# google-deepmind/mujoco_mpc

Measured on NVIDIA H100. Metric: env-steps/sec, higher is better.
Workload: dtype f32

## Files before the change

### mujoco_mpc_b200/csrc/dev_data.cuh

```cuda
#pragma once
#include <cuda_runtime.h>

#include "dev_model.h"

#ifndef MJPC_NO_COMPACT
#define MJPC_COMPACT 1
#endif
#ifdef MJPC_COMPACT
#define MJPC_ROLL _Pragma("unroll 1")
#define MJPC_HESS_ROLLED 1
#else
#define MJPC_ROLL
#endif

namespace mjpc_dev {

constexpr int kMaxSplinePoints = 64;
#define MJPC_D_ARRAYS(X)                                                                                          \
  X(qpos, M.nq) X(qvel, M.nv) X(ctrl, M.nu) X(qacc, M.nv) X(qacc_warmstart, M.nv) X(mocap_pos, 3 * M.nmocap)      \
  X(mocap_quat, 4 * M.nmocap) X(xpos, 3 * M.nbody) X(xquat, 4 * M.nbody) X(xmat, 9 * M.nbody)                     \
  X(xipos, 3 * M.nbody) X(ximat, 9 * M.nbody) X(xanchor, 3 * M.njnt) X(xaxis, 3 * M.njnt)                         \
  X(geom_xpos, 3 * M.ngeom) X(geom_xmat, 9 * M.ngeom) X(site_xpos, 3 * M.nsite) X(subtree_com, 3 * M.nbody)       \
  X(cinert, 10 * M.nbody) X(crb, 10 * M.nbody) X(cdof, 6 * M.nv) X(cdof_dot, 6 * M.nv) X(cvel, 6 * M.nbody)       \
  X(cacc, 6 * M.nbody) X(cfrc, 6 * M.nbody) X(cfrc_sub, 6 * M.nbody) X(subtree_linvel, 3 * M.nbody)               \
// ... 54 lines not shown
  int hdr;
  int lay;
  int ibase;
  int dbase;
  int lane;
  int ncon, nefc, nitem, niter, nlim;
  int ndrow;
  const float* gkey;
  int xfrc_on;
  int npseudo;
  int warn;
  float time;
  unsigned* sync;
  int sync_slot;
  int sync_mode;
#ifdef MJPC_PHASE_TIMING
  long long tph[8], tlast;
#endif
};
#ifdef MJPC_PHASE_TIMING
#define PHASE(c, i) do { const long long t_ = clock64(); (c).tph[i] += t_ - (c).tlast; (c).tlast = t_; } while (0)
#else
#define PHASE(c, i) do { } while (0)
#endif
template <int V> struct IntC { static constexpr int v = V; };
constexpr int kHdrWords = (int)((sizeof(DevModel) + 15) / 16) * 4;
constexpr int kLayWords = (int)((sizeof(DevLayout) + 15) / 16) * 4;

struct DynSpec {
  static constexpr bool kStatic = false;
  static constexpr int kNV = 0, kNHPair = 0;
  static constexpr int kWide = 1, kTask = 0;
  static __device__ __forceinline__ const DevModel& hdr(const Ctx& c) { return *reinterpret_cast<const DevModel*>(g_smem + c.hdr); }
  static __device__ __forceinline__ const DevModel& model(const Ctx& c) { return hdr(c); }
  template <int ID> static __device__ __forceinline__ float* mf(const Ctx& c) { return g_smem + hdr(c).fo[ID]; }
  template <int ID> static __device__ __forceinline__ int* mi(const Ctx& c) {
    return reinterpret_cast<int*>(g_smem + c.ibase) + hdr(c).io[ID];
  }
  template <int ID> static __device__ __forceinline__ float* df(const Ctx& c) {
// ... 22 lines not shown
  template <int ID> static __device__ __forceinline__ int* mi(const Ctx&) {
    return reinterpret_cast<int*>(g_smem) + IntC<View::nf + w(offsetof(DevModel, io), ID)>::v;
  }
  template <int ID> static __device__ __forceinline__ float* df(const Ctx&) {
    return g_smem + IntC<kData0 + K::kLayoutOff[ID]>::v;
  }
};

#define CM(c) (SP::hdr(c))
#define MF(n) (SP::template mf<F_##n>(c))
#define MI(n) (SP::template mi<I_##n>(c))
#define DF(n) (SP::template df<D_##n>(c))
#define DI(n) (reinterpret_cast<int*>(SP::template df<D_##n>(c)))

enum { WIDE_EXIT = 0, WIDE_HESSIAN = 1 };
struct WideBox { int cmd, ncon, nlim, ndrow, nefc; int task_exit, task_warn; float task_cost; };
__device__ __forceinline__ WideBox& wide_box() { __shared__ WideBox box; return box; }
template <class SP>
__device__ __forceinline__ void wide_bar() {
  if constexpr (SP::kWide > 1) asm volatile("bar.sync 1, %0;" ::"n"(32 * SP::kWide) : "memory");
  else __syncwarp();
}
__device__ __forceinline__ void task_bar() { asm volatile("bar.sync 2, 64;" ::: "memory"); }
template <class SP> __device__ __forceinline__ int wide_lane(const Ctx& c) { return SP::kWide > 1 ? (int)threadIdx.x : c.lane; }
template <class SP>
__device__ __forceinline__ void wide_post(const Ctx& c, int cmd) {
  if constexpr (SP::kWide > 1) {
    WideBox& b = wide_box();
    if (c.lane == 0) { b.cmd = cmd; b.ncon = c.ncon; b.nlim = c.nlim; b.ndrow = c.ndrow; b.nefc = c.nefc; }
    wide_bar<SP>();
  }
}

#ifndef MJPC_PAIR_TIMEOUT
#define MJPC_PAIR_TIMEOUT 400000
#endif
constexpr long long kPairTimeout = MJPC_PAIR_TIMEOUT;
__device__ __forceinline__ unsigned ld_vol(const unsigned* p) {
  unsigned v;
  asm volatile("ld.volatile.global.u32 %0, [%1];" : "=r"(v) : "l"(p) : "memory");
  return v;
}
__device__ __forceinline__ void st_vol(unsigned* p, unsigned v) { asm volatile("st.volatile.global.u32 [%0], %1;" ::"l"(p), "r"(v) : "memory"); }
__device__ __forceinline__ void pair_sync_init(Ctx& c, unsigned* table, int mode) {
  c.sync = nullptr; c.sync_slot = -1; c.sync_mode = mode;
// ... 272 lines not shown
```

### mujoco_mpc_b200/csrc/dev_physics.cuh

```cuda
#pragma once
#include "dev_data.cuh"

namespace mjpc_dev {



template <class SP>
__device__ __noinline__ void k_kinematics(Ctx& c) {
  auto&& M = SP::model(c);
  const int lane = c.lane;
  float *xpos = DF(xpos), *xquat = DF(xquat), *xmat = DF(xmat), *xipos = DF(xipos), *ximat = DF(ximat);
  float *xanchor = DF(xanchor), *xaxis = DF(xaxis);
  const float* qpos = DF(qpos);
  if (lane < 3) { xpos[lane] = 0; xipos[lane] = 0; }
  if (lane < 4) xquat[lane] = lane == 0 ? 1.f : 0.f;
  if (lane < 9) { float v = (lane % 4 == 0) ? 1.f : 0.f; xmat[lane] = v; ximat[lane] = v; }
  __syncwarp();
  const int *level_adr = MI(level_adr), *level_body = MI(level_body), *parentid = MI(body_parentid),
            *mocapid = MI(body_mocapid), *jntadr = MI(body_jntadr), *jntnum = MI(body_jntnum),
            *jtype = MI(jnt_type), *jqadr = MI(jnt_qposadr);
  const float *bpos = MF(body_pos), *bquat = MF(body_quat), *bipos = MF(body_ipos), *biquat = MF(body_iquat),
              *jpos = MF(jnt_pos), *jaxis = MF(jnt_axis), *qpos0 = MF(qpos0);
  for (int l = 0; l < M.nlevel; l++) {
    const int a = level_adr[l], e = level_adr[l + 1];
// ... 1108 lines not shown
          FOR_DIM(j, 1, dim) hw[i + j] = Dm * c1 * fr[j - 1] * fr[j - 1];
          float* q = xw + 36 * ci;
          q[0] = mu; q[6] = 0.f;
          FOR_DIM(j, 1, dim) { q[j] = -fr[j - 1] * mu * u[j] * iT; q[6 + j] = fr[j - 1] * u[j]; }
          q[12] = Dm;
          q[13] = Dm * (mu * N * iT * iT * iT - mu * mu * iT * iT);
        }
      }
    }
  }
  cost = warp_sum(cost);
  __syncwarp();
  return cost;
}

template <class SP, int NV, int NQ>
__device__ __forceinline__ void hessian_dense_reg(Ctx& c) {
  auto&& M = SP::model(c);
  const int lane = wide_lane<SP>(c);
  constexpr int WN = 32 * SP::kWide;
  constexpr int NVP = (NV + 3) / 4 * 4;
  const float *qM = DF(qM), *hw = DF(efc_hw), *Jd = DF(efc_Jd), *Xd = DF(efc_Xd), *xw = DF(efc_hc);
  float* H = DF(qH);
  const int *frow = MI(floss_row), *edof = DI(efc_dof), *state = DI(efc_state), *cadr = DI(con_adr),
            *hi = MI(hpair_i), *hj = MI(hpair_j), *cside = DI(con_side), *cdim = DI(con_dim);
  const int NE = M.nhpair, ncon = c.ncon;
  float* Wc = DF(efc_blk);
  float* g = DF(dofbuf);
  const float* W6 = DF(efc_w);
  {
    float* xwm = DF(efc_hc);
    MJPC_ROLL
    for (int w = lane; w < ncon * 6; w += WN) {
      const int ci = w / 6, p = w - 6 * ci;
      const int a0 = cadr[ci];
      float v = 0.f, u = 0.f;
      if (a0 >= 0 && cside[ci] != 0 && state[a0] == STATE_CONE) {
        const int dim = cdim[ci];
        const float* q = xw + 36 * ci;
        FOR_DIM(a, 0, dim) { const float wa = W6[6 * (a0 + a) + p]; v += q[a] * wa; u += q[6 + a] * wa; }
      }
      xwm[36 * ci + 14 + p] = v; xwm[36 * ci + 20 + p] = u;
    }
    wide_bar<SP>();
    constexpr int kMaxRows = 10;
    const bool pyr = M.cone == CONE_PYRAMIDAL;
    const int nwork = ncon * 21;
    MJPC_ROLL
    for (int base = 0; base < nwork; base += WN) {
      const int w = min(base + lane, nwork - 1);
      const int ci = w / 21, e = w - 21 * ci;
      const int p = (e >= 1) + (e >= 3) + (e >= 6) + (e >= 10) + (e >= 15);
      const int q2 = e - p * (p + 1) / 2;
      const int a0r = cadr[ci];
      const bool on = a0r >= 0 && cside[ci] != 0;
      const int a0 = max(a0r, 0);
      const int nrows = on ? cdim[ci] : 0;
      float acc = 0.f;
#ifdef MJPC_HESS_ROLLED
#pragma unroll 1
#else
#pragma unroll
#endif
      for (int a = 0; a < kMaxRows; a++) {
        if (a >= 6 && !pyr) break;
        const int r = min(a0 + a, M.maxefc - 1);
        const float t = hw[r] * W6[6 * r + p] * W6[6 * r + q2];
        acc += a < nrows ? t : 0.f;
      }
      const float* q = xw + 36 * ci;
      const float tc = q[12] * q[14 + p] * q[14 + q2] + q[13] * q[20 + p] * q[20 + q2];
      acc += (on && state[a0] == STATE_CONE) ? tc : 0.f;
      if (base + lane < nwork) Wc[w] = acc;
    }
    wide_bar<SP>();
    const int *subend = MI(body_subtreeend), *cmb = DI(con_mbody), *dbody = MI(dof_bodyid);
    const float* cdof = DF(cdof);
    MJPC_ROLL
    for (int w = lane; w < NV * 6; w += WN) {
      const int i = w / 6, k = w - 6 * i;
      const int b = dbody[i], se = subend[b];
      int idx[6];
      float cd[6];
#pragma unroll
      for (int l = 0; l < 6; l++) { idx[l] = k >= l ? k * (k + 1) / 2 + l : l * (l + 1) / 2 + k; cd[l] = cdof[6 * i + l]; }
      float a = 0.f;
      MJPC_ROLL
      for (int ci = 0; ci < ncon; ci++) {
        const int mb = cmb[ci];
        const float* Wk = Wc + 21 * ci;
        float d = 0.f;
#pragma unroll
        for (int l = 0; l < 6; l++) d += Wk[idx[l]] * cd[l];
        a += (mb >= b && mb < se) ? d : 0.f;
      }
      g[w] = a;
    }
    wide_bar<SP>();
  }
#ifdef MJPC_HESS_ROLLED
  if (NE != NV * (NV + 1) / 2) {
    MJPC_ROLL
    for (int w = lane; w < NV * NV; w += WN) H[w] = 0.f;
    wide_bar<SP>();
  }
  {
    const float* cdof = DF(cdof);
    const int* dbody2 = MI(dof_bodyid);
    const int* drow = DI(efc_drow);
#pragma unroll 1
    for (int e0 = 0; e0 < NE; e0 += WN) {
      const int e = min(e0 + lane, NE - 1);
      const int r = hi[e], sdof = hj[e];
      float a = qM[r * NV + sdof];
      const int br = dbody2[r];
      const unsigned mlo_r = (unsigned)MI(body_dofmask_lo)[br], mhi_r = (unsigned)MI(body_dofmask_hi)[br];
      const bool anc = sdof < 32 ? ((mlo_r >> sdof) & 1u) : ((mhi_r >> (sdof - 32)) & 1u);
      const float *gr = g + 6 * r, *cs = cdof + 6 * sdof;
      float dsum = 0.f;
// ... 14 lines not shown
      }
      if (c.ndrow > 0) {
        MJPC_ROLL
        for (int ci = 0; ci < ncon; ci++) {
          const int a0 = cadr[ci];
          if (a0 < 0 || cside[ci] != 0 || state[a0] != STATE_CONE) continue;
          const float wv = xw[36 * ci + 12], wu = xw[36 * ci + 13];
          const float* xv = Xd + (2 * ci) * NVP;
          const float* xu = xv + NVP;
          a += wv * xv[r] * xv[sdof] + wu * xu[r] * xu[sdof];
        }
      }
      if (e0 + lane < NE) { H[r * NV + sdof] = a; H[sdof * NV + r] = a; }
    }
  }
  wide_bar<SP>();
}
#else
  int er[NQ], es[NQ];
  float acc[NQ];
  for (int w = lane; w < NV * NV; w += 32) H[w] = 0.f;
  {
    const float* cdof = DF(cdof);
    const int* dbody2 = MI(dof_bodyid);
#pragma unroll
    for (int q = 0; q < NQ; q++) {
      int e = lane + 32 * q;
      if (e >= NE) e = NE - 1;
      const int r = hi[e];
      er[q] = r; es[q] = hj[e];
      float a = qM[er[q] * NV + es[q]];
// ... 136 lines not shown
    for (int b0 = 0; b0 < ne; b0 += 32) {
      const int i = min(b0 + lane, ne - 1);
      const float v = j_row_dot<SP>(c, i, nsimple, qacc, nv) - aref[i];
      if (b0 + lane < ne) jar[i] = v;
    }
  }
  g = 0.5f * warp_sum(g);
  __syncwarp();
  const float cc = k_update_constraint<SP>(c, hess);
  *gauss_out = g;
  return cc + g;
}

template <class SP>
__device__ __noinline__ void hessian_static(Ctx& c) {
  hessian_dense_reg<SP, SP::kNV, (SP::kNHPair + 31) / 32>(c);
}

template <class SP>
__device__ __noinline__ void k_hessian(Ctx& c) {
  auto&& M = SP::model(c);
  const int lane = c.lane, nv = M.nv;
  const float *qM = DF(qM), *J = DF(efc_J);
  float *X = DF(efc_W);
  const int *state = DI(efc_state), *cdim = DI(con_dim);
  const float* xw = DF(efc_hc);
  const bool tree_path = SP::kNV > 0 || nv == 18;
  if (!tree_path || c.ndrow > 0) {
    const int *cadr = DI(con_adr), *cnd = DI(con_nd), *cside = DI(con_side);
    const int total = c.ncon * kL;
    for (int w = lane; w < total; w += 32) {
      const int ci = w / kL, l = w - ci * kL;
      const int a0 = cadr[ci];
      if (a0 < 0 || l >= cnd[ci] || state[a0] != STATE_CONE || (tree_path && cside[ci] != 0)) continue;
      const int dim = cdim[ci];
      const float* q = xw + 36 * ci;
      float xv = 0.f, xu = 0.f;
      FOR_DIM(a, 0, dim) {
// ... 8 lines not shown
      const int nvp = (nv + 3) & ~3;
      float* Xd = DF(efc_Xd);
      const int* cloc = DI(con_loc);
      __syncwarp();
      for (int w = lane; w < c.ncon * nv; w += 32) {
        const int ci = w / nv, i = w - ci * nv;
        const int a0 = cadr[ci];
        if (a0 < 0 || state[a0] != STATE_CONE || cside[ci] != 0) continue;
        const int l = cloc[w];
        Xd[(2 * ci) * nvp + i] = l >= 0 ? X[(2 * ci) * kL + l] : 0.f;
        Xd[(2 * ci + 1) * nvp + i] = l >= 0 ? X[(2 * ci + 1) * kL + l] : 0.f;
      }
    }
    __syncwarp();
  }
  if constexpr (SP::kNV > 0) {
    wide_post<SP>(c, WIDE_HESSIAN);
    hessian_static<SP>(c);
    return;
  }
  if (nv == 18 && M.nhpair <= 128) {
    hessian_dense_reg<SP, 18, 4>(c);
  } else if (nv == 18) {
    hessian_dense_reg<SP, 18, 6>(c);
  } else {
    const float *X = DF(efc_W), *hw = DF(efc_hw), *xw = DF(efc_hc);
    float *H = DF(qH), *blk = DF(efc_blk);
    const int *hi = MI(hpair_i), *hj = MI(hpair_j), *frow = MI(floss_row), *state = DI(efc_state), *edof = DI(efc_dof),
              *cadr = DI(con_adr), *cdim = DI(con_dim), *cnd = DI(con_nd), *cloc = DI(con_loc), *cboff = DI(con_boff);
    const int ncon = c.ncon, nf = M.nfloss, nl = c.nlim;
    for (int w = lane; w < nv * nv; w += 32) H[w] = 0.f;
    __syncwarp();
// ... 62 lines not shown
}

template <class SP>
__device__ __noinline__ void wide_helper_loop(Ctx& c) {
  if constexpr (SP::kWide > 1) {
#ifndef MJPC_HESS_ROLLED
    static_assert(SP::kWide == 1, "helper warps need the rolled Hessian assembly (MJPC_COMPACT)");
#endif
    for (;;) {
      wide_bar<SP>();
      const WideBox& b = wide_box();
      const int cmd = b.cmd;
      if (cmd == WIDE_EXIT) return;
      c.ncon = b.ncon; c.nlim = b.nlim; c.ndrow = b.ndrow; c.nefc = b.nefc;
      if (cmd == WIDE_HESSIAN) hessian_static<SP>(c);
    }
  }
}

struct LsPoint { float alpha, cost, d1, d2; };

template <class SP>
__device__ __noinline__ LsPoint k_ls_eval(Ctx& c, float g0, float g1, float g2, float alpha) {
  const int lane = c.lane;
  const float *jar = DF(efc_jar), *Jv = DF(efc_Jv), *D = DF(efc_D), *R = DF(efc_R), *floss = DF(efc_floss);
  const int *etype = DI(efc_type), *eid = DI(efc_id), *item = DI(efc_item), *cdim = DI(con_dim);
  float cost = 0, d1 = 0, d2 = 0;
  for (int it = lane; it < c.nitem; it += 32) {
    const int i = item[it];
    const int ty = etype[i];
// ... 119 lines not shown
#ifdef MJPC_COMPACT
__device__ __noinline__ LsPoint ls_eval_cached_shared(LsItem it, float g0, float g1, float g2, float alpha) {
  return ls_eval_cached(it, g0, g1, g2, alpha);
}
#define LS_EVAL_CACHED ls_eval_cached_shared
#else
#define LS_EVAL_CACHED ls_eval_cached
#endif

template <class SP>
__device__ __noinline__ float k_line_search(Ctx& c, float g0, float g1, float g2, float snorm, float scale_inv) {
  auto&& M = SP::model(c);
  if (snorm < kMinVal) return 0.f;
  const bool cached = c.nitem <= 32;
  const LsItem item = ls_load_item<SP>(c);
  auto ev = [&](float alpha) { return cached ? LS_EVAL_CACHED(item, g0, g1, g2, alpha) : k_ls_eval<SP>(c, g0, g1, g2, alpha); };
  const LsPoint p0 = ev(0.f);
  const float gtol = fmaxf(fmaxf(CM(c).tolerance, kTolFloor) * CM(c).ls_tolerance * snorm * scale_inv, 64 * 1.1920929e-7f * fabsf(p0.d1));
  if (p0.d2 <= kMinVal) return 0.f;
  LsPoint p1 = ev(-p0.d1 / p0.d2);
  if (p0.cost < p1.cost && !(p1.d1 <= 0.f)) p1 = p0;
  if (fabsf(p1.d1) < gtol) return p1.alpha;
  int iter = 0;
  LsPoint p2 = p1;
  bool bracket = false;
  while (iter < M.ls_iterations) {
    iter++;
    p2 = p1;
    if (p1.d2 <= kMinVal) break;
    p1 = ev(p1.alpha - p1.d1 / p1.d2);
    if (fabsf(p1.d1) < gtol) return p1.alpha;
// ... 60 lines not shown
  if constexpr (SP::kNV > 0) jt_force_dense<SP, SP::kNV>(c, out);
  else { if (nv == 18) jt_force_dense<SP, 18>(c, out); else jt_force<SP>(c, out); }
}

template <class SP>
__device__ __noinline__ void k_solve(Ctx& c) {
  auto&& M = SP::model(c);
  const int lane = c.lane, nv = M.nv, ne = c.nefc;
  float *qacc = DF(qacc), *qas = DF(qacc_smooth), *qws = DF(qacc_warmstart), *qfc = DF(qfrc_constraint);
  c.niter = 0;
  if (ne == 0) {
    for (int i = lane; i < nv; i += 32) { qacc[i] = qas[i]; qfc[i] = 0; }
    __syncwarp();
    return;
  }
  float gauss, cost;
  if (!M.disable_warmstart) {
    const float cs = k_total_cost<SP>(c, qas, false, &gauss);
    const float cw = k_total_cost<SP>(c, qws, true, &gauss);
    const bool warm = cw < cs;
    for (int b0 = 0; b0 < nv; b0 += 32) { const int i = min(b0 + lane, nv - 1); const float v = warm ? qws[i] : qas[i]; if (b0 + lane < nv) qacc[i] = v; }
    __syncwarp();
    cost = warm ? cw : k_total_cost<SP>(c, qacc, true, &gauss);
  } else {
    for (int i = lane; i < nv; i += 32) qacc[i] = qas[i];
    __syncwarp();
    cost = k_total_cost<SP>(c, qacc, true, &gauss);
  }
  const float scale_inv = CM(c).meaninertia * (float)max(1, nv);
  const float tol = fmaxf(CM(c).tolerance, kTolFloor);
  const int nsimple = M.nfloss + c.nlim;
  float *grad = DF(grad), *search = DF(search), *Mv = DF(Mv), *Ma = DF(Ma), *smooth = DF(qfrc_smooth), *Jv = DF(efc_Jv),
        *qM = DF(qM);
  float old = cost, prev_gradient = 3.0e38f, alpha = 0.f;
  int stalls = 0;
  bool qfc_current = false;
  for (int iter = 0; iter <= M.iterations; iter++) {
    jt_force_any<SP>(c, qfc, nv);
    qfc_current = true;
    float g2 = 0, ga = 0;
    for (int b0 = 0; b0 < nv; b0 += 32) {
      const int i = min(b0 + lane, nv - 1);
      const bool on = b0 + lane < nv;
      const float a = Ma[i] - smooth[i] - qfc[i];
      if (on) grad[i] = a;
      g2 += on ? a * a : 0.f;
      const float m = fabsf(Ma[i]) + fabsf(smooth[i]) + fabsf(qfc[i]);
      ga += on ? m * m : 0.f;
    }
    const float gnorm2 = warp_sum(g2), gabs2 = warp_sum(ga);
    __syncwarp();
    if (iter > 0) {
      const float improvement = (old - cost) / scale_inv, gradient = sqrtf(gnorm2) / scale_inv;
      const float gfloor = kGradFloor * 1.1920929e-7f * sqrtf(gabs2) / scale_inv;
      if (gradient < fmaxf(tol, gfloor)) break;
      const bool resolvable = fabsf(old - cost) > 16.f * 1.1920929e-7f * fabsf(cost);
      if (resolvable) { if (improvement < tol) break; stalls = 0; }
      else if (gradient > 0.5f * prev_gradient && (alpha > 0.5f || ++stalls >= 3)) break;
      prev_gradient = gradient;
    }
    if (iter == M.iterations) break;
    PHASE(c, 4);
    k_hessian<SP>(c);
    PHASE(c, 5);
    warp_chol_factor_solve<SP::kNV>(DF(qH), DF(hinv), search, grad, nv, lane);
    PHASE(c, 6);
    for (int b0 = 0; b0 < nv; b0 += 32) { const int i = min(b0 + lane, nv - 1); const float v = -search[i]; __syncwarp(); if (b0 + lane < nv) search[i] = v; }
    __syncwarp();
    float q1 = 0, q2 = 0, sn = 0;
    for (int b0 = 0; b0 < nv; b0 += 32) {
      const int i = min(b0 + lane, nv - 1);
      const bool on = b0 + lane < nv;
      const float a = m_row_dot<SP>(qM, i, search, nv);
      if (on) Mv[i] = a;
      const float si = on ? search[i] : 0.f;
      q1 += si * (Ma[i] - smooth[i]);
      q2 += 0.5f * si * a;
      sn += si * si;
    }
    for (int b0 = 0; b0 < ne; b0 += 32) {
      const int i = min(b0 + lane, ne - 1);
      const float v = j_row_dot<SP>(c, i, nsimple, search, nv);
      if (b0 + lane < ne) Jv[i] = v;
    }
    q1 = warp_sum(q1); q2 = warp_sum(q2); sn = sqrtf(warp_sum(sn));
    __syncwarp();
    alpha = k_line_search<SP>(c, gauss, q1, q2, sn, scale_inv);
    if (alpha == 0.f) break;
    for (int b0 = 0; b0 < nv; b0 += 32) { const int i = min(b0 + lane, nv - 1); const float v = qacc[i] + alpha * search[i]; __syncwarp(); if (b0 + lane < nv) qacc[i] = v; }
    __syncwarp();
    old = cost;
    cost = k_total_cost<SP>(c, qacc, true, &gauss, alpha);
    qfc_current = false;
    c.niter = iter + 1;
  }
  if (!qfc_current) jt_force_any<SP>(c, qfc, nv);
}

__device__ __forceinline__ bool k_bad(Ctx& c, const float* v, int n) {
  bool bad = false;
  for (int i = c.lane; i < n; i += 32) bad |= !(fabsf(v[i]) < kMaxVal);
  return __any_sync(kFull, bad);
}

template <class SP>
__device__ __noinline__ void k_forward(Ctx& c) {
  PHASE(c, 7);
  k_kinematics<SP>(c);
  k_com_pos<SP>(c);
  k_crb<SP>(c);
  PHASE(c, 0);
// ... 5 lines not shown
  k_smooth_forces<SP>(c);
  k_reference<SP>(c);
  PHASE(c, 3);
  k_solve<SP>(c);
  PHASE(c, 4);
}

template <class SP>
__device__ __noinline__ void k_euler(Ctx& c) {
  auto&& M = SP::model(c);
  const int lane = c.lane, nv = M.nv;
  const float h = CM(c).timestep;
  float *qacc = DF(qacc), *qvel = DF(qvel), *qpos = DF(qpos), *vt = DF(vtmp);
  const float* acc = qacc;
  if (M.any_damping && !M.disable_eulerdamp) {
    float *H = DF(qH), *qM = DF(qM), *smooth = DF(qfrc_smooth), *qfc = DF(qfrc_constraint);
    const float* damping = MF(dof_damping);
    MJPC_ROLL
    for (int w = lane; w < nv * nv; w += 32) {
      const int r = w / nv, s = w - r * nv;
      H[w] = qM[w] + (r == s ? h * damping[r] : 0.f);
    }
    for (int i = lane; i < nv; i += 32) vt[i] = smooth[i] + qfc[i];
    __syncwarp();
    warp_chol_factor_solve<SP::kNV>(H, DF(hinv), vt, vt, nv, lane);
    acc = vt;
  }
  for (int i = lane; i < nv; i += 32) qvel[i] += h * acc[i];
  __syncwarp();
  const int *jtype = MI(jnt_type), *jqadr = MI(jnt_qposadr), *jdadr = MI(jnt_dofadr);
  for (int j = lane; j < M.njnt; j += 32) {
// ... 17 lines not shown
```

### mujoco_mpc_b200/csrc/rollout_kernels.cuh

```cuda
#pragma once
#include "dev_physics.cuh"
#include "dev_task.cuh"
#include "spec_quadruped.h"
#include "spec_humanoid_track.h"

namespace mjpc_dev {

struct RolloutArgs {
  DevModel M;
  DevLayout L;
  const float* pack;
  int nprob, nper;
  const double* time0;
  const float* state;
  const float* mocap;
  const float* task_state;
  const float* weight;
  const float* parameters;
  const float* knots;
  const float* knot_times;
  FeedbackArgs fb;
  const float* step_sizes;
  int policy_kind;
  float xfrc_std, xfrc_rate;
// ... 40 lines not shown
  const int lay = hdr + (int)((sizeof(DevModel) + 15) / 16) * 4;
  const int data0 = lay + (int)((sizeof(DevLayout) + 15) / 16) * 4;
  {
    const int* srcM = reinterpret_cast<const int*>(M);
    const int* srcL = reinterpret_cast<const int*>(L);
    int* dst = reinterpret_cast<int*>(smem);
    for (int i = threadIdx.x; i < (int)(sizeof(DevModel) / 4); i += blockDim.x) dst[hdr + i] = srcM[i];
    for (int i = threadIdx.x; i < (int)(sizeof(DevLayout) / 4); i += blockDim.x) dst[lay + i] = srcL[i];
  }
  __syncthreads();
  c.hdr = hdr; c.lay = lay; c.ibase = M->nf;
  c.dbase = data0 + warp * L->total;
  c.lane = lane;
  c.gkey = pack + M->nf + M->ni;
  c.ncon = 0; c.npseudo = 0; c.xfrc_on = 0; c.nefc = 0; c.ndrow = 0; c.nitem = 0; c.niter = 0; c.nlim = 0; c.warn = 0; c.time = 0.f;
  c.sync = nullptr; c.sync_slot = -1; c.sync_mode = 0;
#ifdef MJPC_PHASE_TIMING
  for (int k = 0; k < 8; k++) c.tph[k] = 0;
  c.tlast = clock64();
#endif
}

template <class SP>
__device__ __forceinline__ void write_traces(Ctx& c, float* out) {
  auto&& M = SP::model(c);
  const int *ty = MI(task_trace_objtype), *id = MI(task_trace_objid);
  for (int w = c.lane; w < 3 * M.num_trace; w += 32) {
    const int k = w / 3, q = w - 3 * k;
    const float* src = ty[k] == OBJ_SITE ? DF(site_xpos) : ty[k] == OBJ_GEOM ? DF(geom_xpos) : ty[k] == OBJ_XBODY ? DF(xpos) : DF(xipos);
    out[w] = src[3 * id[k] + q];
  }
}

// ... 7 lines not shown
    c0 = n0; c1 = lo1; c2 = n2; c3 = lo0;
    k0 += 0x9E3779B9u; k1 += 0xBB67AE85u;
  }
  const float u1 = ((float)c0 + 0.5f) * 2.3283064365386963e-10f, u2 = ((float)c1 + 0.5f) * 2.3283064365386963e-10f;
  return sqrtf(-2.0f * logf(fmaxf(u1, 1e-12f))) * cospif(2.0f * u2);
}

template <class SP>
__device__ __noinline__ void task_warp_loop(Ctx& c, const RolloutArgs& A, int cand) {
  auto&& M = SP::model(c);
  const int lane = c.lane, nu = M.nu, nr = M.num_residual, ntr = 3 * M.num_trace, H = A.H;
  (void)nu;
  c.xfrc_on = A.xfrc_std > 0.f ? 1 : 0;
  float* o_res = A.residual + (size_t)cand * H * nr;
  float* o_trace = A.trace + (size_t)cand * H * ntr;
  for (int t = 0; t < H; t++) {
    const bool last = t == H - 1;
    task_bar();
    if (wide_box().task_exit) return;
    k_crb<SP>(c);
    k_com_vel<SP>(c);
    k_smooth_forces<SP>(c);
    task_bar();
    k_residual<SP>(c);
    for (int i = lane; i < nr; i += 32) o_res[(size_t)t * nr + i] = DF(residual)[i];
    write_traces<SP>(c, o_trace + (size_t)t * ntr);
    const float cost = k_cost_value<SP>(c);
    if (lane == 0) { wide_box().task_cost = cost; wide_box().task_warn = c.warn; }
    if (!last) {
      c.time += CM(c).timestep;
      if (A.policy_kind == 0 && t + 1 < H - 1) k_policy_spline<SP>(c, A.P, A.interp);
    }
    task_bar();
  }
}

template <class SP>
// ... 72 lines not shown
      o_actions[(size_t)t * nu + i] = DF(ctrl)[i];
    }
    if (!last && (k_bad(c, DF(qpos), nq) || k_bad(c, DF(qvel), nv))) {
      failed = true;
      if (kTask) { if (lane == 0) wide_box().task_exit = 1; task_bar(); }
      break;
    }
    if (noisy && !last) {
      float* xf = DF(xfrc);
      for (int i = lane; i < 6 * M.nbody; i += 32)
        xf[i] = ou_rate * xf[i] + ou_scale * xfrc_normal(A.noise_seed, (unsigned)t, (unsigned)(A.cand0 + cand), (unsigned)i);
      __syncwarp();
    }
    float cost;
    if constexpr (kTask) {
      PHASE(c, 7);
      k_kinematics<SP>(c);
      k_com_pos<SP>(c);
      PHASE(c, 0);
      task_bar();
      k_collision<SP>(c);
      PHASE(c, 1);
      k_make_constraint<SP>(c);
      PHASE(c, 2);
      task_bar();
      k_reference<SP>(c);
      PHASE(c, 3);
      if (c.sync_mode & 2) pair_sync_meet(c, 2 * t + 1);
      k_solve<SP>(c);
      PHASE(c, 4);
      n_newton += c.niter; n_con += c.ncon - c.npseudo; n_efc += c.nefc;
      if (!last && k_bad(c, DF(qacc), nv)) c.warn = 1;
      task_bar();
      cost = wide_box().task_cost;
      if (wide_box().task_warn) c.warn = 1;
    } else {
      k_forward<SP>(c);
      n_newton += c.niter; n_con += c.ncon - c.npseudo; n_efc += c.nefc;
      k_residual<SP>(c);
      if (!last && k_bad(c, DF(qacc), nv)) c.warn = 1;
      for (int i = lane; i < nr; i += 32) o_res[(size_t)t * nr + i] = DF(residual)[i];
      write_traces<SP>(c, o_trace + (size_t)t * ntr);
    }
    if (c.warn) {
      failed = true;
      if (kTask && !last) { if (lane == 0) wide_box().task_exit = 1; task_bar(); }
      break;
    }
    if constexpr (!kTask) cost = k_cost_value<SP>(c);
    if (lane == 0) o_costs[t] = cost;
    total += cost;
    if (last) break;
    for (int i = lane; i < nv; i += 32) DF(qacc_warmstart)[i] = DF(qacc)[i];
    k_euler<SP>(c);
    for (int i = lane; i < nq; i += 32) o_states[(size_t)(t + 1) * ds + i] = DF(qpos)[i];
    for (int i = lane; i < nv; i += 32) o_states[(size_t)(t + 1) * ds + nq + i] = DF(qvel)[i];
    if (lane == 0) o_times[t + 1] = time0 + (double)c.time;
  }
  pair_sync_done(c);
  wide_post<SP>(c, WIDE_EXIT);
  if (lane == 0) {
    A.returns[cand] = failed ? 1.0e6f : total / (float)max(H, 1);
    A.failure[cand] = failed ? 1 : 0;
    if (A.stats) {
      A.stats[12 * cand] = clock64() - clk0; A.stats[12 * cand + 1] = n_newton;
      A.stats[12 * cand + 2] = n_con; A.stats[12 * cand + 3] = n_efc;
      for (int k = 0; k < 8; k++) {
#ifdef MJPC_PHASE_TIMING
        A.stats[12 * cand + 4 + k] = c.tph[k];
#else
        A.stats[12 * cand + 4 + k] = 0;
#endif
      }
#ifndef MJPC_PHASE_TIMING
      unsigned smid, warpid;
      asm volatile("mov.u32 %0, %%smid;" : "=r"(smid));
      asm volatile("mov.u32 %0, %%warpid;" : "=r"(warpid));
      A.stats[12 * cand + 4] = smid; A.stats[12 * cand + 5] = warpid;
#endif
    }
  }
}

extern "C" __global__ void __launch_bounds__(128) rollout_kernel(const __grid_constant__ RolloutArgs A) {
  rollout_body<DynSpec>(A);
}
#ifndef MJPC_WIDE
#define MJPC_WIDE 6
#endif
#ifndef MJPC_TASK
#define MJPC_TASK 1
#endif
constexpr int kRolloutWide = MJPC_WIDE, kRolloutTask = MJPC_TASK, kRolloutThreads = 32 * (kRolloutWide + kRolloutTask);
extern "C" __global__ void __launch_bounds__(kRolloutThreads) rollout_kernel_quadruped(const __grid_constant__ RolloutArgs A) {
  rollout_body<StaticSpec<SpecQuadruped, kRolloutWide, kRolloutTask>>(A);
}
extern "C" __global__ void __launch_bounds__(32) rollout_kernel_quadruped_plain(const __grid_constant__ RolloutArgs A) {
  rollout_body<StaticSpec<SpecQuadruped, 1, 0>>(A);
}
extern "C" __global__ void __launch_bounds__(kRolloutThreads) rollout_kernel_humanoid_track(const __grid_constant__ RolloutArgs A) {
  rollout_body<StaticSpec<SpecHumanoidTrack, kRolloutWide, kRolloutTask>>(A);
}
extern "C" __global__ void __launch_bounds__(32) rollout_kernel_humanoid_track_plain(const __grid_constant__ RolloutArgs A) {
// ... 142 lines not shown
```

### profiles/phase_times.py

```python
import os, sys
import numpy as np
R = os.path.dirname(os.path.dirname(os.path.abspath(__file__))); sys.path.insert(0, R); sys.path.insert(0, os.path.join(R, "tests"))
from conftest import get_model, quadruped_inputs
from mujoco_mpc_b200.engine import Engine
m = get_model("quadruped")
e = Engine(m, 256, 64)
d = np.load(os.path.join(R, "profiles", "inputs_quadruped_256x64.npz"))
state, mocap, knots, kt = d["state"], d["mocap"], d["knots"], d["kt"]
for _ in range(2):
    e.rollout_spline(state, 0.0, mocap, knots, kt, 2, 64)
st = e.fetch_stats().astype(float)
tot = st[:, 0]
names = ["kinematics+com+crb", "collision", "make_constraint", "vel+smooth+reference", "solve (rest)", "solve: Hessian assembly", "solve: Cholesky factor+solve", "policy+residual+cost+euler+output"]
print("kernel %.2f ms; per-candidate cycles median %.3g" % (e.last_kernel_ms, np.median(tot)))
for k, n in enumerate(names):
    if n != "-":
        print("  %-36s %5.1f%% of cycles  (%.0f cycles/step)" % (n, 100 * st[:, 4 + k].sum() / tot.sum(), st[:, 4 + k].mean() / 64))
print("  newton iterations/step %.2f  -> cycles per Newton iteration: all of solve %.0f, Hessian %.0f, Cholesky %.0f" % (
    st[:, 1].mean() / 64, st[:, 8:11].sum() / st[:, 1].sum(), st[:, 9].sum() / st[:, 1].sum(), st[:, 10].sum() / st[:, 1].sum()))
```

### profiles/sanitize.py

```python
import os, sys
import numpy as np
R = os.path.dirname(os.path.dirname(os.path.abspath(__file__))); sys.path.insert(0, R); sys.path.insert(0, os.path.join(R, "tests"))
from conftest import get_model, mocap_of, quadruped_inputs
from mujoco_mpc_b200.engine import Engine
from mujoco_mpc_b200.ilqg import ILQGPlanner
which = sys.argv[1] if len(sys.argv) > 1 else "all"
m = get_model("quadruped")
e = Engine(m, 8, 12)
state, mocap, knots, kt = quadruped_inputs(m, N=4, H=10)
if which in ("all", "rollout"):
    for shape in ("wide", "plain"):
        os.environ["MJPC_B200_SHAPE"] = shape
        e.rollout_spline(state, 0.0, mocap, knots, kt, 2, 10)
        assert e.last_kernel_shape == (1 if shape == "wide" else 2)
    del os.environ["MJPC_B200_SHAPE"]
    os.environ["MJPC_B200_NO_STATIC"] = "1"
    e.rollout_spline(state, 0.0, mocap, knots, kt, 2, 10)
    del os.environ["MJPC_B200_NO_STATIC"]
    e.set_xfrc_noise(1.0, 0.1, 3); e.rollout_spline(state, 0.0, mocap, knots, kt, 2, 10); e.set_xfrc_noise(0.0)
if which in ("all", "ilqg"):
    pl = ILQGPlanner(m, e, horizon=8, num_rollouts=4, fd_tolerance=1e-3)
    pl.set_state(state, 0.0, mocap)
    pl.optimize_policy()
if which in ("all", "humanoid"):
    mh = get_model("humanoid_track")
    eh = Engine(mh, 4, 10)
    mc = np.concatenate([mh.key_mpos[0].reshape(-1, 3), np.tile([1.0, 0, 0, 0], (mh.nmocap, 1))], 1).reshape(-1)
    sh = np.concatenate([mh.key_qpos[0], np.zeros(mh.nv)])
    kh = np.clip(0.1 * np.random.default_rng(0).standard_normal((2, 16, mh.nu)), -1, 1)
    for shape in ("wide", "plain"):
# ... 9 lines not shown
```

Before: 2.497 million.

## Assemble Newton Hessian on helper warps asynchronously, overlapping gradient and line search

In wide kernels the main warp now computes cone rows, posts a Hessian command with a non-blocking barrier arrive, and carries on with J^T f, the gradient and termination checks. Helper warps (wide minus one) assemble the dense Hessian and signal completion on a separate named barrier, and the main warp joins only before the Cholesky step. The default wide count goes from 6 to 7 so the helper group keeps the same number of warps. Euler damping uses qLD as scratch instead of qH to avoid racing with the helpers. This also adds extra phase-timing maps for profiling. It risks extra warps per block lowering occupancy, and Hessian work is wasted on the final iteration when it exits early.

```diff
diff --git a/mujoco_mpc_b200/csrc/dev_data.cuh b/mujoco_mpc_b200/csrc/dev_data.cuh
--- a/mujoco_mpc_b200/csrc/dev_data.cuh
+++ b/mujoco_mpc_b200/csrc/dev_data.cuh
@@ -92,15 +92,20 @@
   unsigned* sync;
   int sync_slot;
   int sync_mode;
+  int wide_pending;
 #ifdef MJPC_PHASE_TIMING
-  long long tph[8], tlast;
-#endif
-};
+  long long tph[9], tlast;
+#endif
+};
+#ifndef MJPC_PHASE_MAP
+#define MJPC_PHASE_MAP 0
+#endif
 #ifdef MJPC_PHASE_TIMING
-#define PHASE(c, i) do { const long long t_ = clock64(); (c).tph[i] += t_ - (c).tlast; (c).tlast = t_; } while (0)
+#define PHASE_AT(c, m, i) do { if (MJPC_PHASE_MAP == (m)) { const long long t_ = clock64(); (c).tph[i] += t_ - (c).tlast; (c).tlast = t_; } } while (0)
 #else
-#define PHASE(c, i) do { } while (0)
-#endif
+#define PHASE_AT(c, m, i) do { } while (0)
+#endif
+#define PHASE(c, i) PHASE_AT(c, 0, i)
 template <int V> struct IntC { static constexpr int v = V; };
 constexpr int kHdrWords = (int)((sizeof(DevModel) + 15) / 16) * 4;
 constexpr int kLayWords = (int)((sizeof(DevLayout) + 15) / 16) * 4;
@@ -153,7 +158,12 @@
 #define DI(n) (reinterpret_cast<int*>(SP::template df<D_##n>(c)))
 
 enum { WIDE_EXIT = 0, WIDE_HESSIAN = 1 };
-struct WideBox { int cmd, ncon, nlim, ndrow, nefc; int task_exit, task_warn; float task_cost; };
+struct WideBox {
+  int cmd, ncon, nlim, ndrow, nefc; int task_exit, task_warn; float task_cost;
+#ifdef MJPC_PHASE_TIMING
+  long long task_fork_cycles;
+#endif
+};
 __device__ __forceinline__ WideBox& wide_box() { __shared__ WideBox box; return box; }
 template <class SP>
 __device__ __forceinline__ void wide_bar() {
@@ -162,12 +172,39 @@
 }
 __device__ __forceinline__ void task_bar() { asm volatile("bar.sync 2, 64;" ::: "memory"); }
 template <class SP> __device__ __forceinline__ int wide_lane(const Ctx& c) { return SP::kWide > 1 ? (int)threadIdx.x : c.lane; }
+template <class SP, bool kHelpers>
+struct WideGroup {
+  static constexpr int kWarps = kHelpers ? SP::kWide - 1 : SP::kWide;
+  static __device__ __forceinline__ int lane(const Ctx& c) { return kHelpers ? (int)threadIdx.x - 32 : wide_lane<SP>(c); }
+  static __device__ __forceinline__ void bar() {
+    if constexpr (!kHelpers) wide_bar<SP>();
+    else if constexpr (kWarps > 1) asm volatile("bar.sync 4, %0;" ::"n"(32 * kWarps) : "memory");
+    else __syncwarp();
+  }
+};
 template <class SP>
 __device__ __forceinline__ void wide_post(const Ctx& c, int cmd) {
   if constexpr (SP::kWide > 1) {
     WideBox& b = wide_box();
     if (c.lane == 0) { b.cmd = cmd; b.ncon = c.ncon; b.nlim = c.nlim; b.ndrow = c.ndrow; b.nefc = c.nefc; }
     wide_bar<SP>();
+  }
+}
+template <class SP>
+__device__ __forceinline__ void wide_post_async(const Ctx& c, int cmd) {
+  static_assert(SP::kWide > 1, "a one-warp trajectory has no helpers to post to");
+  WideBox& b = wide_box();
+  if (c.lane == 0) { b.cmd = cmd; b.ncon = c.ncon; b.nlim = c.nlim; b.ndrow = c.ndrow; b.nefc = c.nefc; }
+  asm volatile("bar.arrive 1, %0;" ::"n"(32 * SP::kWide) : "memory");
+}
+template <class SP>
+__device__ __forceinline__ void wide_join() { asm volatile("bar.sync 3, %0;" ::"n"(32 * SP::kWide) : "memory"); }
+template <class SP>
+__device__ __forceinline__ void wide_done() { asm volatile("bar.arrive 3, %0;" ::"n"(32 * SP::kWide) : "memory"); }
+template <class SP>
+__device__ __forceinline__ void wide_settle(Ctx& c) {
+  if constexpr (SP::kWide > 1) {
+    if (c.wide_pending) { wide_join<SP>(); c.wide_pending = 0; }
   }
 }
 
diff --git a/mujoco_mpc_b200/csrc/dev_physics.cuh b/mujoco_mpc_b200/csrc/dev_physics.cuh
--- a/mujoco_mpc_b200/csrc/dev_physics.cuh
+++ b/mujoco_mpc_b200/csrc/dev_physics.cuh
@@ -1146,11 +1146,12 @@
   return cost;
 }
 
-template <class SP, int NV, int NQ>
+template <class SP, int NV, int NQ, bool kHelpers = false>
 __device__ __forceinline__ void hessian_dense_reg(Ctx& c) {
   auto&& M = SP::model(c);
-  const int lane = wide_lane<SP>(c);
-  constexpr int WN = 32 * SP::kWide;
+  using G = WideGroup<SP, kHelpers>;
+  const int lane = G::lane(c);
+  constexpr int WN = 32 * G::kWarps;
   constexpr int NVP = (NV + 3) / 4 * 4;
   const float *qM = DF(qM), *hw = DF(efc_hw), *Jd = DF(efc_Jd), *Xd = DF(efc_Xd), *xw = DF(efc_hc);
   float* H = DF(qH);
@@ -1174,7 +1175,7 @@
       }
       xwm[36 * ci + 14 + p] = v; xwm[36 * ci + 20 + p] = u;
     }
-    wide_bar<SP>();
+    G::bar();
     constexpr int kMaxRows = 10;
     const bool pyr = M.cone == CONE_PYRAMIDAL;
     const int nwork = ncon * 21;
@@ -1205,7 +1206,7 @@
       acc += (on && state[a0] == STATE_CONE) ? tc : 0.f;
       if (base + lane < nwork) Wc[w] = acc;
     }
-    wide_bar<SP>();
+    G::bar();
     const int *subend = MI(body_subtreeend), *cmb = DI(con_mbody), *dbody = MI(dof_bodyid);
     const float* cdof = DF(cdof);
     MJPC_ROLL
@@ -1228,13 +1229,13 @@
       }
       g[w] = a;
     }
-    wide_bar<SP>();
+    G::bar();
   }
 #ifdef MJPC_HESS_ROLLED
   if (NE != NV * (NV + 1) / 2) {
     MJPC_ROLL
     for (int w = lane; w < NV * NV; w += WN) H[w] = 0.f;
-    wide_bar<SP>();
+    G::bar();
   }
   {
     const float* cdof = DF(cdof);
@@ -1279,7 +1280,7 @@
       if (e0 + lane < NE) { H[r * NV + sdof] = a; H[sdof * NV + r] = a; }
     }
   }
-  wide_bar<SP>();
+  G::bar();
 }
 #else
   int er[NQ], es[NQ];
@@ -1446,14 +1447,14 @@
 
 template <class SP>
 __device__ __noinline__ void hessian_static(Ctx& c) {
-  hessian_dense_reg<SP, SP::kNV, (SP::kNHPair + 31) / 32>(c);
-}
-
-template <class SP>
-__device__ __noinline__ void k_hessian(Ctx& c) {
+  hessian_dense_reg<SP, SP::kNV, (SP::kNHPair + 31) / 32, (SP::kWide > 1)>(c);
+}
+
+template <class SP>
+__device__ __forceinline__ void hessian_cone_rows(Ctx& c) {
   auto&& M = SP::model(c);
   const int lane = c.lane, nv = M.nv;
-  const float *qM = DF(qM), *J = DF(efc_J);
+  const float* J = DF(efc_J);
   float *X = DF(efc_W);
   const int *state = DI(efc_state), *cdim = DI(con_dim);
   const float* xw = DF(efc_hc);
@@ -1492,8 +1493,16 @@
     }
     __syncwarp();
   }
+}
+
+template <class SP>
+__device__ __noinline__ void k_hessian(Ctx& c) {
+  auto&& M = SP::model(c);
+  const int lane = c.lane, nv = M.nv;
+  const float *qM = DF(qM), *J = DF(efc_J);
+  hessian_cone_rows<SP>(c);
   if constexpr (SP::kNV > 0) {
-    wide_post<SP>(c, WIDE_HESSIAN);
+    static_assert(SP::kWide == 1, "helper-warp kernels assemble on the helpers (k_solve)");
     hessian_static<SP>(c);
     return;
   }
@@ -1586,6 +1595,7 @@
       if (cmd == WIDE_EXIT) return;
       c.ncon = b.ncon; c.nlim = b.nlim; c.ndrow = b.ndrow; c.nefc = b.nefc;
       if (cmd == WIDE_HESSIAN) hessian_static<SP>(c);
+      wide_done<SP>();
     }
   }
 }
@@ -1735,7 +1745,12 @@
   if (snorm < kMinVal) return 0.f;
   const bool cached = c.nitem <= 32;
   const LsItem item = ls_load_item<SP>(c);
-  auto ev = [&](float alpha) { return cached ? LS_EVAL_CACHED(item, g0, g1, g2, alpha) : k_ls_eval<SP>(c, g0, g1, g2, alpha); };
+  auto ev = [&](float alpha) {
+#if defined(MJPC_PHASE_TIMING) && MJPC_PHASE_MAP == 1
+    c.tph[7]++;
+#endif
+    return cached ? LS_EVAL_CACHED(item, g0, g1, g2, alpha) : k_ls_eval<SP>(c, g0, g1, g2, alpha);
+  };
   const LsPoint p0 = ev(0.f);
   const float gtol = fmaxf(fmaxf(CM(c).tolerance, kTolFloor) * CM(c).ls_tolerance * snorm * scale_inv, 64 * 1.1920929e-7f * fabsf(p0.d1));
   if (p0.d2 <= kMinVal) return 0.f;
@@ -1826,6 +1841,7 @@
     __syncwarp();
     return;
   }
+  PHASE_AT(c, 1, 8);
   float gauss, cost;
   if (!M.disable_warmstart) {
     const float cs = k_total_cost<SP>(c, qas, false, &gauss);
@@ -1839,6 +1855,7 @@
     __syncwarp();
     cost = k_total_cost<SP>(c, qacc, true, &gauss);
   }
+  PHASE_AT(c, 1, 4);
   const float scale_inv = CM(c).meaninertia * (float)max(1, nv);
   const float tol = fmaxf(CM(c).tolerance, kTolFloor);
   const int nsimple = M.nfloss + c.nlim;
@@ -1848,6 +1865,14 @@
   int stalls = 0;
   bool qfc_current = false;
   for (int iter = 0; iter <= M.iterations; iter++) {
+    if constexpr (SP::kWide > 1) {
+      if (iter < M.iterations) {
+        hessian_cone_rows<SP>(c);
+        wide_post_async<SP>(c, WIDE_HESSIAN);
+        c.wide_pending = 1;
+        PHASE_AT(c, 1, 5);
+      }
+    }
     jt_force_any<SP>(c, qfc, nv);
     qfc_current = true;
     float g2 = 0, ga = 0;
@@ -1871,12 +1896,16 @@
       else if (gradient > 0.5f * prev_gradient && (alpha > 0.5f || ++stalls >= 3)) break;
       prev_gradient = gradient;
     }
+    PHASE_AT(c, 1, 0);
     if (iter == M.iterations) break;
     PHASE(c, 4);
-    k_hessian<SP>(c);
+    if constexpr (SP::kWide > 1) wide_settle<SP>(c);
+    else k_hessian<SP>(c);
     PHASE(c, 5);
+    PHASE_AT(c, 1, 5);
     warp_chol_factor_solve<SP::kNV>(DF(qH), DF(hinv), search, grad, nv, lane);
     PHASE(c, 6);
+    PHASE_AT(c, 1, 6);
     for (int b0 = 0; b0 < nv; b0 += 32) { const int i = min(b0 + lane, nv - 1); const float v = -search[i]; __syncwarp(); if (b0 + lane < nv) search[i] = v; }
     __syncwarp();
     float q1 = 0, q2 = 0, sn = 0;
@@ -1897,7 +1926,9 @@
     }
     q1 = warp_sum(q1); q2 = warp_sum(q2); sn = sqrtf(warp_sum(sn));
     __syncwarp();
+    PHASE_AT(c, 1, 1);
     alpha = k_line_search<SP>(c, gauss, q1, q2, sn, scale_inv);
+    PHASE_AT(c, 1, 2);
     if (alpha == 0.f) break;
     for (int b0 = 0; b0 < nv; b0 += 32) { const int i = min(b0 + lane, nv - 1); const float v = qacc[i] + alpha * search[i]; __syncwarp(); if (b0 + lane < nv) qacc[i] = v; }
     __syncwarp();
@@ -1905,8 +1936,11 @@
     cost = k_total_cost<SP>(c, qacc, true, &gauss, alpha);
     qfc_current = false;
     c.niter = iter + 1;
-  }
+    PHASE_AT(c, 1, 3);
+  }
+  PHASE_AT(c, 1, 0);
   if (!qfc_current) jt_force_any<SP>(c, qfc, nv);
+  PHASE_AT(c, 1, 0);
 }
 
 __device__ __forceinline__ bool k_bad(Ctx& c, const float* v, int n) {
@@ -1942,7 +1976,7 @@
   float *qacc = DF(qacc), *qvel = DF(qvel), *qpos = DF(qpos), *vt = DF(vtmp);
   const float* acc = qacc;
   if (M.any_damping && !M.disable_eulerdamp) {
-    float *H = DF(qH), *qM = DF(qM), *smooth = DF(qfrc_smooth), *qfc = DF(qfrc_constraint);
+    float *H = SP::kWide > 1 ? DF(qLD) : DF(qH), *qM = DF(qM), *smooth = DF(qfrc_smooth), *qfc = DF(qfrc_constraint);
     const float* damping = MF(dof_damping);
     MJPC_ROLL
     for (int w = lane; w < nv * nv; w += 32) {
diff --git a/mujoco_mpc_b200/csrc/rollout_kernels.cuh b/mujoco_mpc_b200/csrc/rollout_kernels.cuh
--- a/mujoco_mpc_b200/csrc/rollout_kernels.cuh
+++ b/mujoco_mpc_b200/csrc/rollout_kernels.cuh
@@ -78,9 +78,9 @@
   c.lane = lane;
   c.gkey = pack + M->nf + M->ni;
   c.ncon = 0; c.npseudo = 0; c.xfrc_on = 0; c.nefc = 0; c.ndrow = 0; c.nitem = 0; c.niter = 0; c.nlim = 0; c.warn = 0; c.time = 0.f;
-  c.sync = nullptr; c.sync_slot = -1; c.sync_mode = 0;
+  c.sync = nullptr; c.sync_slot = -1; c.sync_mode = 0; c.wide_pending = 0;
 #ifdef MJPC_PHASE_TIMING
-  for (int k = 0; k < 8; k++) c.tph[k] = 0;
+  for (int k = 0; k < 9; k++) c.tph[k] = 0;
   c.tlast = clock64();
 #endif
 }
@@ -118,13 +118,23 @@
   c.xfrc_on = A.xfrc_std > 0.f ? 1 : 0;
   float* o_res = A.residual + (size_t)cand * H * nr;
   float* o_trace = A.trace + (size_t)cand * H * ntr;
+#ifdef MJPC_PHASE_TIMING
+  long long fork_cycles = 0;
+#endif
   for (int t = 0; t < H; t++) {
     const bool last = t == H - 1;
     task_bar();
     if (wide_box().task_exit) return;
+#ifdef MJPC_PHASE_TIMING
+    const long long t_fork = clock64();
+#endif
     k_crb<SP>(c);
     k_com_vel<SP>(c);
     k_smooth_forces<SP>(c);
+#ifdef MJPC_PHASE_TIMING
+    fork_cycles += clock64() - t_fork;
+    if (lane == 0) wide_box().task_fork_cycles = fork_cycles;
+#endif
     task_bar();
     k_residual<SP>(c);
     for (int i = lane; i < nr; i += 32) o_res[(size_t)t * nr + i] = DF(residual)[i];
@@ -227,21 +237,23 @@
     }
     float cost;
     if constexpr (kTask) {
-      PHASE(c, 7);
+      PHASE(c, 7); PHASE_AT(c, 2, 7);
+      wide_settle<SP>(c);
       k_kinematics<SP>(c);
       k_com_pos<SP>(c);
-      PHASE(c, 0);
+      PHASE(c, 0); PHASE_AT(c, 2, 0);
       task_bar();
       k_collision<SP>(c);
-      PHASE(c, 1);
+      PHASE(c, 1); PHASE_AT(c, 2, 1);
       k_make_constraint<SP>(c);
-      PHASE(c, 2);
+      PHASE(c, 2); PHASE_AT(c, 2, 2);
       task_bar();
+      PHASE_AT(c, 2, 3);
       k_reference<SP>(c);
       PHASE(c, 3);
       if (c.sync_mode & 2) pair_sync_meet(c, 2 * t + 1);
       k_solve<SP>(c);
-      PHASE(c, 4);
+      PHASE(c, 4); PHASE_AT(c, 2, 4);
       n_newton += c.niter; n_con += c.ncon - c.npseudo; n_efc += c.nefc;
       if (!last && k_bad(c, DF(qacc), nv)) c.warn = 1;
       task_bar();
@@ -271,6 +283,7 @@
     if (lane == 0) o_times[t + 1] = time0 + (double)c.time;
   }
   pair_sync_done(c);
+  wide_settle<SP>(c);
   wide_post<SP>(c, WIDE_EXIT);
   if (lane == 0) {
     A.returns[cand] = failed ? 1.0e6f : total / (float)max(H, 1);
@@ -278,6 +291,9 @@
     if (A.stats) {
       A.stats[12 * cand] = clock64() - clk0; A.stats[12 * cand + 1] = n_newton;
       A.stats[12 * cand + 2] = n_con; A.stats[12 * cand + 3] = n_efc;
+#if defined(MJPC_PHASE_TIMING) && MJPC_PHASE_MAP == 2
+      if constexpr (kTask) c.tph[5] = wide_box().task_fork_cycles;
+#endif
       for (int k = 0; k < 8; k++) {
 #ifdef MJPC_PHASE_TIMING
         A.stats[12 * cand + 4 + k] = c.tph[k];
@@ -299,7 +315,7 @@
   rollout_body<DynSpec>(A);
 }
 #ifndef MJPC_WIDE
-#define MJPC_WIDE 6
+#define MJPC_WIDE 7
 #endif
 #ifndef MJPC_TASK
 #define MJPC_TASK 1
diff --git a/profiles/phase_times.py b/profiles/phase_times.py
--- a/profiles/phase_times.py
+++ b/profiles/phase_times.py
@@ -1,8 +1,11 @@
-import os, sys
+import argparse, os, sys
 import numpy as np
 R = os.path.dirname(os.path.dirname(os.path.abspath(__file__))); sys.path.insert(0, R); sys.path.insert(0, os.path.join(R, "tests"))
 from conftest import get_model, quadruped_inputs
 from mujoco_mpc_b200.engine import Engine
+ap = argparse.ArgumentParser()
+ap.add_argument("--map", type=int, default=0, choices=[0, 1, 2])
+args = ap.parse_args()
 m = get_model("quadruped")
 e = Engine(m, 256, 64)
 d = np.load(os.path.join(R, "profiles", "inputs_quadruped_256x64.npz"))
@@ -11,10 +14,25 @@
     e.rollout_spline(state, 0.0, mocap, knots, kt, 2, 64)
 st = e.fetch_stats().astype(float)
 tot = st[:, 0]
-names = ["kinematics+com+crb", "collision", "make_constraint", "vel+smooth+reference", "solve (rest)", "solve: Hessian assembly", "solve: Cholesky factor+solve", "policy+residual+cost+euler+output"]
+NAMES = {
+    0: ["kinematics+com+crb", "collision", "make_constraint", "vel+smooth+reference", "solve (rest)", "solve: Hessian assembly",
+        "solve: Cholesky factor+solve", "policy+residual+cost+euler+output"],
+    1: ["J^T f + gradient + termination", "M/J products", "line search", "step + constraint update", "warm-start evaluations",
+        "Hessian (assembly, or post + join wait)", "Cholesky factor + solve", "-"],
+    2: ["kinematics+com", "collision", "make_constraint", "wait at join 1", "reference + solve", "-", "-", "rest of the step"],
+}[args.map]
 print("kernel %.2f ms; per-candidate cycles median %.3g" % (e.last_kernel_ms, np.median(tot)))
-for k, n in enumerate(names):
+for k, n in enumerate(NAMES):
     if n != "-":
-        print("  %-36s %5.1f%% of cycles  (%.0f cycles/step)" % (n, 100 * st[:, 4 + k].sum() / tot.sum(), st[:, 4 + k].mean() / 64))
-print("  newton iterations/step %.2f  -> cycles per Newton iteration: all of solve %.0f, Hessian %.0f, Cholesky %.0f" % (
-    st[:, 1].mean() / 64, st[:, 8:11].sum() / st[:, 1].sum(), st[:, 9].sum() / st[:, 1].sum(), st[:, 10].sum() / st[:, 1].sum()))
+        print("  %-40s %5.1f%% of cycles  (%.0f cycles/step)" % (n, 100 * st[:, 4 + k].sum() / tot.sum(), st[:, 4 + k].mean() / 64))
+if args.map == 0:
+    print("  newton iterations/step %.2f  -> cycles per Newton iteration: all of solve %.0f, Hessian %.0f, Cholesky %.0f" % (
+        st[:, 1].mean() / 64, st[:, 8:11].sum() / st[:, 1].sum(), st[:, 9].sum() / st[:, 1].sum(), st[:, 10].sum() / st[:, 1].sum()))
+elif args.map == 1:
+    rest = tot - st[:, 4:11].sum(1)
+    print("  %-40s %5.1f%% of cycles  (%.0f cycles/step)" % ("outside the solve", 100 * rest.sum() / tot.sum(), rest.mean() / 64))
+    print("  newton iterations/step %.2f, line-search evaluations/step %.2f (%.2f per iteration)" % (
+        st[:, 1].mean() / 64, st[:, 11].mean() / 64, st[:, 11].sum() / st[:, 1].sum()))
+else:
+    print("  %-40s %5s   (%.0f cycles/step; the main warp's collision + constraint rows: %.0f)" % (
+        "task warp: CRB+velocities+smooth forces", "", st[:, 9].mean() / 64, st[:, 5:7].sum(1).mean() / 64))
diff --git a/profiles/sanitize.py b/profiles/sanitize.py
--- a/profiles/sanitize.py
+++ b/profiles/sanitize.py
@@ -14,6 +14,8 @@
         e.rollout_spline(state, 0.0, mocap, knots, kt, 2, 10)
         assert e.last_kernel_shape == (1 if shape == "wide" else 2)
     del os.environ["MJPC_B200_SHAPE"]
+    mt = type(m)(m); mt.opt_tolerance = 1.0
+    et = Engine(mt, 8, 12); et.rollout_spline(state, 0.0, mocap, knots, kt, 2, 10); et.close()
     os.environ["MJPC_B200_NO_STATIC"] = "1"
     e.rollout_spline(state, 0.0, mocap, knots, kt, 2, 10)
     del os.environ["MJPC_B200_NO_STATIC"]
```

Result: faster. 2.572 million (median of 6 runs) (+3.0%).
